# jeun-990806/pim-jpeg-decoder

Measured on AMD Instinct MI355X. Metric: MPixels/sec JPEG->RGB (bit-exact BMP), higher is better.
Workload: dtype int16/int32 (integer IDCT), u8 out

## Files before the change

### pim-jpeg-decoder_amd/csrc/pjd_k_huffman.hip

```cpp
#include <cstdlib>

#include "pjd_device_common.h"
#include "pjd_kernels.h"
#include "pjd_lut_build.h"
#include "../../include/pjd.h"

static_assert(sizeof(PjdDevHuffRaw) == 180, "raw table layout");
static_assert(PJD_LUT_BITS + PJD_L2_BITS == 16 && PJD_L1_BYTES == (4 << PJD_LUT_BITS), "two-level table geometry");
static_assert(PJD_HUFF_LANES == 64, "one wave per 64 lanes");
static_assert(PJD_STAGE_ENTRIES == PJD_GROUP && PJD_GROUP == 16, "a group (a head word + 7 step words) is what one flush of the staging buffer writes");

__global__ __launch_bounds__(256) void pjd_k_build_tables(PjdDevBatch B)
{
    const uint32_t ts = blockIdx.x / PJD_MAX_TABLES, slot = blockIdx.x % PJD_MAX_TABLES;
    const PjdDevTset &T = B.tsets[ts];
    if (slot >= T.n_tables || T.lut_bytes == 0) return;
    const PjdDevHuffRaw &r = B.raw_tables[(size_t)ts * PJD_MAX_TABLES + slot];
    uint16_t *blob = reinterpret_cast<uint16_t *>(B.luts + (size_t)T.lut_off16 * 16);
    uint32_t *L1 = reinterpret_cast<uint32_t *>(blob + slot * (PJD_L1_BYTES / 2));
    const uint32_t partner = r.is_ac ? slot : (uint32_t)T.pair_ac[slot];
    const bool has_partner = partner < T.n_tables;
    const PjdDevHuffRaw &r2 = B.raw_tables[(size_t)ts * PJD_MAX_TABLES + (has_partner ? partner : slot)];
    __shared__ uint32_t first[17], first2[17];
    __shared__ uint16_t cp[PJD_L2_BITS], ce[PJD_L2_BITS];
// ... 16 lines not shown

struct __attribute__((packed)) UnalignedU32x4 { uint32_t v[4]; };

__global__ __launch_bounds__(256) void pjd_k_lane_words(PjdDevBatch B)
{
    const uint32_t wv = blockIdx.x;
    const PjdDevHuffWave hw = B.hwaves[wv];
    const PjdDevImage &im = B.images[hw.image];
    const uint32_t l = threadIdx.x & 63, k0 = threadIdx.x >> 6;
    const uint32_t rows = PJD_WORD_ROWS(im.sub_bytes);
    uint32_t *dst = B.words + (size_t)wv * B.word_rows * 64;
    const bool valid = l < hw.n_lanes;
    const uint8_t *src = B.ecs + im.ecs_off + (valid ? B.lanes[hw.first_lane + l].byte_start : 0u);
#if PJD_WORDS_X4
    for (uint32_t k = 4 * k0; k < rows; k += 16) {
        uint32_t w[4] = {0, 0, 0, 0};
        if (valid) {
            const UnalignedU32x4 v = *reinterpret_cast<const UnalignedU32x4 *>(src + 4 * k);
#pragma unroll
            for (int j = 0; j < 4; j++) w[j] = __builtin_bswap32(v.v[j]);
        }
#pragma unroll
        for (int j = 0; j < 4; j++) dst[(k + j) * 64 + l] = w[j];
    }
#else
    for (uint32_t k = k0; k < rows; k += 4) {
        uint32_t w = 0;
        if (valid) w = __builtin_bswap32(reinterpret_cast<const UnalignedU32 *>(src + 4 * k)->v);
        dst[k * 64 + l] = w;
    }
#endif
}

typedef const __attribute__((address_space(1))) uint8_t *pjd_gptr;
#if PJD_DIRECT_ECS
#define PJD_WORD_STRIDE 4u
#else
#define PJD_WORD_STRIDE 256u
#endif
struct BitWin {
    pjd_gptr wb;
    uint32_t hi, lo, nxt;
    uint32_t off;
    int s;
    __device__ __forceinline__ uint32_t word(uint32_t byte_off) const
    {
#if PJD_DIRECT_ECS
        return __builtin_bswap32(reinterpret_cast<const __attribute__((address_space(1))) UnalignedU32 *>(wb + byte_off)->v);
#else
        return *reinterpret_cast<const __attribute__((address_space(1))) uint32_t *>(wb + byte_off);
#endif
    }
    __device__ __forceinline__ void init(pjd_gptr wave_words, uint32_t col, uint32_t p)
    {
        wb = wave_words;
        const int kk = (int)((p + 31) >> 5) - 1;
        const uint32_t o = (uint32_t)(kk + 1) * PJD_WORD_STRIDE + col;
        hi = kk >= 0 ? word(o - PJD_WORD_STRIDE) : 0u;
        lo = word(o);
        nxt = word(o + PJD_WORD_STRIDE);
        off = o + 2 * PJD_WORD_STRIDE;
        s = 32 * (kk + 1) - (int)p;
    }
    __device__ __forceinline__ uint32_t peek() const { return __builtin_amdgcn_alignbit(hi, lo, (uint32_t)s); }
    __device__ __forceinline__ void drop(uint32_t n)
    {
// ... 78 lines not shown
    __device__ __forceinline__ void build(uint32_t lane) const
    {
        if (lane <= dus1) {
            const uint32_t rn = next(lane), cn = comp(rn);
            uint4 rec;
            rec.x = tabs(rn);
            rec.y = xbase + rn * 16;
            rec.z = cn == 0 ? 0x0000ffffu : (cn == 1 ? 0xffff0000u : 0u);
            rec.w = cn == 2 ? 0x0000ffffu : 0u;
            pjd_v4u32 v; v.x = rec.x; v.y = rec.y; v.z = rec.z; v.w = rec.w;
            *reinterpret_cast<__attribute__((address_space(3))) pjd_v4u32 *>(xbase + lane * 16) = v;
        }
    }
    __device__ __forceinline__ uint32_t self(uint32_t r) const { return xbase + (r == dus1 ? 0u : r + 1) * 16; }
};

struct ChkCtx {
    uint32_t *state;
    uint32_t *rem;
    uint32_t chk_bits;
    uint32_t walk_max;
};

enum { SPAN_END = 0, SPAN_MERGED = 1, SPAN_MERGED_B = 2 };

struct BCache {
    uint32_t st;
    uint32_t rem;
    uint32_t p, cz;
};

__device__ __forceinline__ void chk_finish(const ChkCtx &K, uint32_t j, uint32_t ndu)
{
    for (uint32_t i = 1; i < j; i++) K.rem[i * 64] = ndu - K.rem[i * 64];
}

__device__ __forceinline__ uint32_t lut_lookup_pair(uint32_t lbase, uint32_t tab, uint32_t pk)
{
    uint32_t e = lds_u32(tab + 4 * __builtin_amdgcn_ubfe(pk, 32 - PJD_LUT_BITS, PJD_LUT_BITS));
    if (__builtin_expect(PJD_LUT_USED(e) == 0, 0)) {
        e = lds_u16(lbase + PJD_LUT_PTR_BYTES(e) + 2u * ((pk << PJD_LUT_BITS) >> PJD_LUT_PTR_SHIFT(e)));
        e |= e << 16;
    }
    return e;
}
__device__ __forceinline__ uint32_t lut_lookup(uint32_t lbase, uint32_t tab, uint32_t pk) { return lut_lookup_pair(lbase, tab, pk) & 0xffffu; }

__device__ __forceinline__ uint32_t rfl(uint32_t v) { return (uint32_t)__builtin_amdgcn_readfirstlane((int)v); }

__device__ __forceinline__ uint32_t add_flag(uint32_t v, bool f)
{
    uint32_t d;
    asm("v_addc_co_u32_e64 %0, vcc, %1, 0, %2" : "=v"(d) : "v"(v), "s"(__builtin_amdgcn_ballot_w64(f)) : "vcc");
    return d;
}

template <bool BRIDGE>
__device__ __forceinline__ int sync_span(const PhaseCtx &P, pjd_gptr wave_words, uint32_t col,
                                         uint32_t &p, uint32_t &c, uint32_t &z, uint32_t end_bit,
                                         uint32_t &ndu, const ChkCtx &K, uint32_t &jout, uint32_t Bst, uint32_t &oldA_st, uint32_t &oldA_rem)
{
    uint32_t j = 1;
    jout = 1;
    oldA_st = 0xffffffffu; oldA_rem = 0;
    if (p >= end_bit) return SPAN_END;
    BitWin2 w;
    w.init(wave_words, col, p);
    uint32_t ra, x;
    {
        const uint2 cur = lds_u32x2(P.self(P.dus1 - c));
        x = cur.x; ra = cur.y;
    }
    int zb = 63 - (int)z;
    uint32_t next_chk = K.chk_bits;
    uint32_t lim = next_chk < end_bit ? next_chk : end_bit;
    int res = SPAN_END;
    auto step = [&](uint32_t pk) -> bool {
        const uint2 nx = lds_u32x2(ra);
        const uint32_t tab = (zb == 63) ? (x & 0xffffu) : (x >> 16);
        const uint32_t e = lut_lookup_pair(P.lbase, tab, pk);
        const uint32_t u1 = PJD_LUT_USED(e), u12 = PJD_LUT_PAIR_USED(e);
// ... 134 lines not shown
            st = (63u << 8) | (st & 0xffu);
            if ((st & 0x80u) || second) break;
            second = true; Ddc = DdcB; Dac = DacB; Edc = e2; Eac = e3;
        }
#undef WALK_FIX
#undef WALK_PTR
        zb = (int)(st >> 8);
        const uint32_t k = (st & 0xffu) - bias;
        p += k;
        if (p >= lim) {
            if (p >= end_bit) break;
            const uint32_t st = (p << 14) | (r << 10) | (uint32_t)zb;
            const uint32_t a = rfl(st_col[j * 64]);
            if (a == st) { ndu += rfl(rem_col[j * 64]); res = SPAN_MERGED; break; }
            if (j == 1) {
                oldA_st = a; oldA_rem = rfl(rem_col[64]);
                if (st == Bst) { res = SPAN_MERGED_B; break; }
            }
            if (l == 0) { st_col[j * 64] = st; rem_col[j * 64] = ndu; }
            j++;
            next_chk += chk_bits;
            lim = next_chk < end_bit ? next_chk : end_bit;
        }
    }
    c = dus1 - r;
    z = 63u - (uint32_t)zb;
    jout = j;
    return res;
#undef WALK_TABS
#undef WALK_NEXT
}

struct OutCtx {
    uint16_t *region;
    uint32_t *stage;
    uint32_t cap;
    uint32_t n;
    uint32_t npair;
    uint32_t dcA, dcB;
    uint32_t mark_D;
    uint32_t ru;
    PjdDevMark *marks;
    uint32_t mark_next;
    uint32_t lane_q;
    uint32_t overflow;
    uint32_t D_in;
};

__device__ __forceinline__ void stage_flush(const OutCtx &O, uint32_t first_slot)
{
    uint4 *dst = reinterpret_cast<uint4 *>(O.region + first_slot);
#pragma unroll
    for (int k = 0; k < PJD_STAGE_ENTRIES / 8; k++) {
        uint4 v;
        v.x = O.stage[(4 * k + 0) * 64]; v.y = O.stage[(4 * k + 1) * 64];
        v.z = O.stage[(4 * k + 2) * 64]; v.w = O.stage[(4 * k + 3) * 64];
        dst[k] = v;
    }
}

struct WState {
    uint32_t p;
    int zb;
    uint32_t ra, x;
    uint32_t mA, mB;
    uint32_t emax;
    uint32_t umin;
};

typedef unsigned short pjd_u16x2 __attribute__((ext_vector_type(2)));
__device__ __forceinline__ uint32_t pk_add16(uint32_t a, uint32_t b)
{
    return __builtin_bit_cast(uint32_t, (pjd_u16x2)(__builtin_bit_cast(pjd_u16x2, a) + __builtin_bit_cast(pjd_u16x2, b)));
}

__device__ __forceinline__ int jpeg_extend(uint32_t bits, uint32_t size)
{
    const uint32_t m1 = 1u << size;
    return (int)bits + ((((int)bits - (int)(m1 >> 1)) >> 31) & (int)(1u - m1));
}
__device__ __forceinline__ int jpeg_value(uint32_t pk, uint32_t used, uint32_t size)
{
    const uint32_t off = 32u - used;
    const uint32_t b = __builtin_amdgcn_ubfe(pk, off, size);
    const uint32_t m = (1u << size) - 1u;
    const uint32_t top = (uint32_t)__builtin_amdgcn_sbfe(pk, off + size - 1u, 1u);
    return (int)(b - (m & ~top));
}

template <bool FIRST>
__device__ __forceinline__ uint32_t write_step(uint32_t lbase, BitWin2 &w, WState &S, uint32_t &D, OutCtx &O, uint32_t end_bit)
{
    const bool is_dc = (S.zb == 63);
    if (__builtin_expect(is_dc && D == O.mark_D, 0)) {
        PjdDevMark m;
        m.lane = O.lane_q; m.ent_off = O.n;
        m.acc[0] = (uint16_t)O.dcA; m.acc[1] = (uint16_t)(O.dcA >> 16); m.acc[2] = (uint16_t)O.dcB; m.pad_ = 0;
        O.marks[O.mark_next++] = m;
        O.mark_D += O.ru;
    }
    const uint32_t pk = FIRST ? w.peek0() : w.peek1();
    const uint4 nx = lds_u32x4(S.ra);
    const uint32_t tab = is_dc ? (S.x & 0xffffu) : (S.x >> 16);
    const uint32_t e = lut_lookup_pair(lbase, tab, pk);
    const uint32_t u1 = PJD_LUT_USED(e), size1 = PJD_LUT_SIZE(e), adv1 = PJD_LUT_ADV(e);
    const uint32_t u12 = PJD_LUT_PAIR_USED(e), adv12 = PJD_LUT_PAIR_ADV(e), size2 = PJD_LUT_PAIR_SIZE2(e);
    const bool pair = u12 != u1 && S.zb >= (int)adv1 && S.p + u1 < end_bit;
    O.npair += pair ? 1u : 0u;
    const int val1 = jpeg_value(pk, u1, size1);
    const int val2 = jpeg_value(pk, u12, size2);
    const uint32_t used = pair ? u12 : u1, adv = pair ? adv12 : adv1;
    w.drop(used);
    S.p += used;
    { const uint32_t el = e & 0xffffu; S.emax = S.emax > el ? S.emax : el; }
    S.zb -= (int)adv;
    const bool done = S.zb < 0;
    { const uint32_t u = (uint32_t)(S.zb + 16); S.umin = S.umin < u ? S.umin : u; }
    const uint32_t entA = is_dc ? (uint32_t)val1 : (((uint32_t)val1 << 5) | (adv1 & 31u));
    const uint32_t entB = pair ? (((uint32_t)val2 << 5) | ((adv12 - adv1) & 31u)) : PJD_ENT_NONE;
    const uint32_t dv = is_dc ? ((uint32_t)val1 & 0xffffu) : 0u;
    const uint32_t dvv = dv | (dv << 16);
    O.dcA = pk_add16(O.dcA, dvv & S.mA);
    O.dcB = pk_add16(O.dcB, dvv & S.mB);
    S.zb = done ? 63 : S.zb;
    S.ra = done ? nx.y : S.ra;
    S.x = done ? nx.x : S.x;
    S.mA = done ? nx.z : S.mA;
    S.mB = done ? nx.w : S.mB;
    D = add_flag(D, done);
// ... 54 lines not shown
    uint32_t dcA, dcB;
};

__device__ __forceinline__ void careful_span(const PhaseCtx &P, pjd_gptr wave_words, uint32_t col, uint32_t p, uint32_t c, uint32_t z,
                                          uint32_t end_bit, uint32_t eof_rel, bool to_eof, uint32_t D, uint32_t D_end, uint16_t *region, uint32_t cap,
                                          Careful &R)
{
    const uint32_t D_in = D;
    uint32_t *region32 = reinterpret_cast<uint32_t *>(region);
    BitWin w;
    w.init(wave_words, col, p);
    uint4 cur = lds_u32x4(P.self(P.dus1 - c));
    int zb = 63 - (int)z;
    R.n = 0; R.ovf = 0; R.cls = 0; R.p_err = 0; R.D_err = 0; R.in_dc = 0; R.dcA = 0; R.dcB = 0;
    const bool at_end = eof_rel != 0xffffffffu;
    bool open = false;
    uint32_t open_at = 0, open_ent = 0;
    while (D < D_end && (p < end_bit || to_eof)) {
        const bool is_dc = zb == 63;
        if (!open) {
            if ((R.n & (PJD_GROUP - 1)) == 0 && R.n + 2 <= cap) {
                region32[R.n >> 1] = ((D - D_in) << 8) | (63u - (uint32_t)zb);
                R.n += 2;
            }
            if (is_dc && D == R.mark_D) {
                PjdDevMark m;
                m.lane = R.lane_q; m.ent_off = R.n;
                m.acc[0] = (uint16_t)R.dcA; m.acc[1] = (uint16_t)(R.dcA >> 16); m.acc[2] = (uint16_t)R.dcB; m.pad_ = 0;
                R.marks[R.mark_next++] = m;
                R.mark_D += R.ru;
            }
        }
        const uint32_t pk = w.peek();
        const uint4 nx = lds_u32x4(cur.y);
        const uint32_t e = lut_lookup(P.lbase, is_dc ? (cur.x & 0xffffu) : (cur.x >> 16), pk);
        const uint32_t used = PJD_LUT_USED(e), size = PJD_LUT_SIZE(e), adv = PJD_LUT_ADV(e);
        const uint32_t vbits = size >= PJD_LUT_BADSYM ? 0u : size, codelen = used - vbits;
        const uint32_t left = !at_end ? 64u : (eof_rel > p ? eof_rel - p : 0u);
        uint32_t bad = 0;
        if (size == PJD_LUT_BADSYM || codelen > left) bad = is_dc ? PJD_ST_DC_SYM : PJD_ST_AC_SYM;
        else if (is_dc) {
            if (size == PJD_LUT_BADLEN) bad = PJD_ST_DC_LEN;
            else if (vbits > left - codelen) bad = PJD_ST_DC_BITS;
        } else if (!(e & PJD_LUT_EOB)) {
            if (zb - (int)adv <= -2) bad = PJD_ST_AC_RUN;
            else if (size == PJD_LUT_BADLEN) bad = PJD_ST_AC_LEN;
            else if (vbits > left - codelen) bad = PJD_ST_AC_BITS;
        }
        if (bad) {
            R.cls = bad; R.p_err = p; R.D_err = D; R.in_dc = is_dc ? 1u : 0u;
            if (!is_dc) {
                if (open) region32[open_at] = open_ent | (PJD_ENT_EOB << 16);
                else if (R.n + 2 <= cap) { region32[R.n >> 1] = PJD_ENT_EOB | (PJD_ENT_NONE << 16); R.n += 2; }
                else R.ovf = 1;
            }
            break;
        }
        const int val = jpeg_extend(__builtin_amdgcn_ubfe(pk, 32u - used, size), size);
        w.drop(used);
        p += used;
        zb -= (int)adv;
        const bool done = zb < 0;
        const uint32_t ent = is_dc ? ((uint32_t)val & 0xffffu) : ((((uint32_t)val << 5) | (adv & 31u)) & 0xffffu);
        if (open) { region32[open_at] = open_ent | (ent << 16); open = false; }
        else if (R.n + 2 <= cap) {
            region32[R.n >> 1] = ent | (PJD_ENT_NONE << 16);
            open = !done; open_at = R.n >> 1; open_ent = ent;
            R.n += 2;
        } else R.ovf = 1;
        const uint32_t dv = is_dc ? ((uint32_t)val & 0xffffu) : 0u, dvv = dv | (dv << 16);
        R.dcA = pk_add16(R.dcA, dvv & cur.z);
        R.dcB = pk_add16(R.dcB, dvv & cur.w);
        if (done) { zb = 63; cur = nx; D++; }
    }
    if ((R.n & (PJD_GROUP - 1)) == 2) R.n -= 2;
}

struct LaneGeom {
    bool valid, seg_first, seg_last;
    uint32_t q;
    uint32_t seg;
    uint32_t end_bit;
    uint32_t seg_end_bit;
    uint32_t base_bit;
    pjd_gptr words;
    uint32_t col;
};

extern __shared__ __attribute__((aligned(16))) uint8_t pjd_huff_lds[];

struct WaveState { uint32_t p_img, cz, cnt; };

__device__ __forceinline__ bool wave_rounds(const PhaseCtx &P, const LaneGeom &g, const ChkCtx &K, WalkBuf &wb, WaveState &S, BCache &Bc, uint32_t changed,
                                            uint32_t ext_p, uint32_t ext_cz, bool ext_new, uint32_t &err_acc,
                                            unsigned long long *stats, int stat_base, uint32_t *rdbg)
{
    const uint32_t l = threadIdx.x & 63;
    for (int iter = 0; iter < PJD_SYNC_MAX_ITERS; iter++) {
#if PJD_TAIL_PRIO
        if (iter == 1) __builtin_amdgcn_s_setprio(2);
        if (iter == 4) __builtin_amdgcn_s_setprio(3);
#endif
        uint32_t pp = __shfl_up(S.p_img, 1), pcz = __shfl_up(S.cz, 1), pch = __shfl_up(changed, 1);
        if (l == 0) { pp = ext_p; pcz = ext_cz; pch = (ext_new && iter == 0) ? 1u : 0u; }
        const bool act = g.valid && !g.seg_first && pch != 0;
        const uint64_t act_mask = __ballot(act);
        if (!act_mask) return true;
        const uint64_t tr0 = rdbg ? __builtin_amdgcn_s_memrealtime() : 0;
        if ((uint32_t)__popcll(act_mask) <= K.walk_max) {
            uint64_t mask = act_mask;
            uint32_t walked = 0;
            const uint32_t chk_bits = rfl(K.chk_bits);
            const uint64_t can = __ballot(g.valid && !g.seg_first);
            while (mask) {
                uint32_t a = (uint32_t)__builtin_ctzll(mask);
                mask &= mask - 1;
                uint32_t ep = rfl(ext_p), ecz = rfl(ext_cz);
                if (a) { ep = (uint32_t)__builtin_amdgcn_readlane((int)S.p_img, (int)(a - 1)); ecz = (uint32_t)__builtin_amdgcn_readlane((int)S.cz, (int)(a - 1)); }
                for (;;) {
                    const uint32_t base = (uint32_t)__builtin_amdgcn_readlane((int)g.base_bit, (int)a);
                    const uint32_t endb = (uint32_t)__builtin_amdgcn_readlane((int)g.end_bit, (int)a);
                    uint32_t p = ep - base, c = ecz >> 8, z = ecz & 255u, ndu = 0, j;
                    uint32_t *st_col = K.state - l + a, *rem_col = K.rem - l + a;
                    const uint32_t Bst_a = (uint32_t)__builtin_amdgcn_readlane((int)Bc.st, (int)a);
                    uint32_t oa_st, oa_rem;
                    const int res = walk_lane(P, wb, l, base, p, c, z, endb, ndu, st_col, rem_col, chk_bits, j, Bst_a, oa_st, oa_rem);
                    walked++;
                    const uint32_t op = (uint32_t)__builtin_amdgcn_readlane((int)S.p_img, (int)a), ocz = (uint32_t)__builtin_amdgcn_readlane((int)S.cz, (int)a);
                    uint32_t np = p + base, ncz = (c << 8) | z;
                    if (res == SPAN_MERGED_B) {
                        const uint32_t Brem_a = (uint32_t)__builtin_amdgcn_readlane((int)Bc.rem, (int)a);
                        np = (uint32_t)__builtin_amdgcn_readlane((int)Bc.p, (int)a); ncz = (uint32_t)__builtin_amdgcn_readlane((int)Bc.cz, (int)a);
                        ndu += Brem_a;
                        if (l == 0) { st_col[64] = Bst_a; rem_col[64] = Brem_a; st_col[128] = 0xffffffffu; st_col[192] = 0xffffffffu; }
                    } else if (l == 0) for (uint32_t i = 1; i < j; i++) rem_col[i * 64] = ndu - rem_col[i * 64];
                    if (l == a) {
                        S.cnt = ndu;
                        if (oa_st != 0xffffffffu || res == SPAN_MERGED_B) { Bc.st = oa_st; Bc.rem = oa_rem; Bc.p = op; Bc.cz = ocz; }
                    }
                    if (res == SPAN_MERGED || (np == op && ncz == ocz)) break;
                    if (l == a) { S.p_img = np; S.cz = ncz; }
                    if (a == 63) break;
                    if (!((can >> (a + 1)) & 1ull)) break;
                    a++; mask &= ~(1ull << a);
                    ep = np; ecz = ncz;
                }
            }
            if (stats && l == 0) { atomicAdd(stats + stat_base, 1ull); atomicAdd(stats + stat_base + 1, (unsigned long long)walked); atomicAdd(stats + PJD_STAT_WALKS, 1ull); atomicAdd(stats + PJD_STAT_WALKS + 1, (unsigned long long)walked); }
            if (rdbg && l == 0 && iter < 24) rdbg[iter] = ((0x80u | (walked & 0x7fu)) << 24) | ((uint32_t)(__builtin_amdgcn_s_memrealtime() - tr0) & 0xffffffu);
            return true;
        }
        if (stats && l == 0) { atomicAdd(stats + stat_base, 1ull); atomicAdd(stats + stat_base + 1, (unsigned long long)__popcll(act_mask)); }
        changed = 0;
        if (act) {
            uint32_t p = pp - g.base_bit, c = pcz >> 8, z = pcz & 255, ndu = 0, j, oa_st, oa_rem;
            const int res = sync_span<true>(P, g.words, g.col, p, c, z, g.end_bit, ndu, K, j, Bc.st, oa_st, oa_rem);
            const uint32_t op = S.p_img, ocz = S.cz;
            if (res == SPAN_MERGED_B) {
                ndu += Bc.rem;
                K.state[64] = Bc.st; K.rem[64] = Bc.rem; K.state[128] = 0xffffffffu; K.state[192] = 0xffffffffu;
                if (Bc.p != S.p_img || Bc.cz != S.cz) { S.p_img = Bc.p; S.cz = Bc.cz; changed = 1; }
            } else {
                chk_finish(K, j, ndu);
                if (res != SPAN_MERGED) {
                    const uint32_t np = p + g.base_bit, ncz = (c << 8) | z;
                    if (np != S.p_img || ncz != S.cz) { S.p_img = np; S.cz = ncz; changed = 1; }
                }
            }
// ... 139 lines not shown
            const uint32_t i1 = i0 + PJD_HUFF_THREADS, i2 = i1 + PJD_HUFF_THREADS, i3 = i2 + PJD_HUFF_THREADS;
            uint4 v0 = tsrc[i0], v1, v2, v3;
            if (i1 < n16) v1 = tsrc[i1];
            if (i2 < n16) v2 = tsrc[i2];
            if (i3 < n16) v3 = tsrc[i3];
            tdst[i0] = v0;
            if (i1 < n16) tdst[i1] = v1;
            if (i2 < n16) tdst[i2] = v2;
            if (i3 < n16) tdst[i3] = v3;
        }
    }
    const bool wave_on = wi < wg.n_waves;
    const uint32_t w = wg.first_wave + (wave_on ? wi : 0u);
    const PjdDevHuffWave hw = B.hwaves[w];
    const PjdDevImage &im = B.images[hw.image];
    PhaseCtx P;
    {
        const uint32_t nl = rfl(im.n_luma), dus = rfl(im.dus_per_mcu), nc = dus - nl;
        const uint32_t c1 = nc >= 1 ? 1u : 0u, c2 = nc >= 2 ? 2u : c1;
        const uint32_t lb = lds_abs(lds);
        P.lbase = lb;
        P.tY  = rfl((lb + (uint32_t)im.tbl_slot[0][0] * PJD_L1_BYTES) | (lb + (uint32_t)im.tbl_slot[0][1] * PJD_L1_BYTES) << 16);
        P.tC1 = rfl((lb + (uint32_t)im.tbl_slot[c1][0] * PJD_L1_BYTES) | (lb + (uint32_t)im.tbl_slot[c1][1] * PJD_L1_BYTES) << 16);
        P.tC2 = rfl((lb + (uint32_t)im.tbl_slot[c2][0] * PJD_L1_BYTES) | (lb + (uint32_t)im.tbl_slot[c2][1] * PJD_L1_BYTES) << 16);
        P.nc = nc; P.dus1 = dus - 1;
        P.xbase = lds_abs(phase_tabs) + wi * PJD_PHASE_LDS;
    }
    const uint32_t dus = P.dus1 + 1;
    P.build(l);
    __syncthreads();
    if (!wave_on) return;
    if (B.pull) __builtin_amdgcn_s_setprio(1);

    const uint64_t ts0 = B.dbg ? __builtin_amdgcn_s_memrealtime() : 0;
    const uint64_t tc0 = B.dbg ? __builtin_amdgcn_s_memtime() : 0;
    uint64_t *genA = B.wave_gen, *genB = B.wave_gen + B.n_hwave;
    LaneGeom g;
    g.valid = l < hw.n_lanes;
    g.q = hw.first_lane + l;
    g.seg_first = g.seg_last = false;
    g.seg = 0; g.end_bit = g.seg_end_bit = g.base_bit = 0;
#if PJD_DIRECT_ECS
    g.words = (pjd_gptr)readfirstlane_u64((uint64_t)(B.ecs + im.ecs_off));
    g.col = 0;
#else
    g.words = (pjd_gptr)readfirstlane_u64((uint64_t)(B.words + (size_t)w * B.word_rows * 64));
    g.col = l * 4;
#endif
    uint32_t seg_first_du = 0, seg_n_du = 0;
    const uint32_t sub_bytes = rfl(im.sub_bytes);
    if (g.valid) {
        const PjdDevSub sb = B.lanes[g.q];
        g.seg = sb.seg & 0x7fffffffu;
        g.seg_first = (sb.seg >> 31) != 0;
        const PjdDevSegment sg = B.segs[g.seg];
        const uint32_t end_byte = sb.byte_start + sub_bytes < sg.byte_end ? sb.byte_start + sub_bytes : sg.byte_end;
        g.seg_last = end_byte == sg.byte_end;
        g.base_bit = sb.byte_start * 8;
#if PJD_DIRECT_ECS
        g.col = sb.byte_start;
#endif
        g.end_bit = (end_byte - sb.byte_start) * 8;
        g.seg_end_bit = (sg.byte_end - sb.byte_start) * 8;
        seg_first_du = sg.first_du; seg_n_du = sg.n_du;
    }
    uint32_t *area = reinterpret_cast<uint32_t *>(areas + wi * PJD_WAVE_LDS);
    ChkCtx K;
    K.state = area + l;
    K.rem = area + PJD_NCHK * 64 + l;
    K.chk_bits = sub_bytes * 8 / PJD_NCHK;
    K.walk_max = rfl(im.walk_max);
    for (int j = 0; j < PJD_NCHK; j++) { K.state[j * 64] = 0xffffffffu; K.rem[j * 64] = 0; }
    const bool first_is_head = __shfl((uint32_t)g.seg_first, 0) != 0;
    const uint32_t last_lane = hw.n_lanes - 1;
    bool dead = false;
    uint32_t flag = 0;

    WaveState S;
    {
        uint32_t p = 0, c = 0, z = 0, ndu = 0, j = 1;
        if (g.valid) {
            uint32_t oa, orem;
            sync_span<false>(P, g.words, g.col, p, c, z, g.end_bit, ndu, K, j, 0xffffffffu, oa, orem);
            chk_finish(K, j, ndu);
        }
        S.p_img = p + g.base_bit; S.cz = (c << 8) | z; S.cnt = ndu;
    }
    if (l == last_lane) op_store(genA + w, pjd_pack_state(S.p_img, S.cz >> 8, S.cz & 255) | OP_FLAG);
    const uint64_t ts1 = B.dbg ? __builtin_amdgcn_s_memrealtime() : 0;

    uint64_t entry_used = 0;
    uint32_t err_acc = 0;
    bool ok = true;
    WalkBuf wb;
    wb.ecs = (pjd_gptr)readfirstlane_u64((uint64_t)(B.ecs + im.ecs_off));
    wb.clamp = rfl(im.ecs_len) + 40u;
    wb.cb = 0; wb.cw = 0; wb.cn = 0; wb.have = 0;
    if (!first_is_head) entry_used = op_wait_flag(genA + w - 1, dead);
    BCache Bc;
    Bc.st = 0xffffffffu; Bc.rem = 0; Bc.p = 0; Bc.cz = 0;
    ok = wave_rounds(P, g, K, wb, S, Bc, g.valid ? 1u : 0u, (uint32_t)entry_used,
                     (((uint32_t)(entry_used >> 32) & 255) << 8) | ((uint32_t)(entry_used >> 40) & 255), !first_is_head && !dead,
                     err_acc, B.stats, 0, B.dbg ? B.dbg + (size_t)w * 32 + 8 : nullptr);
    if (l == last_lane) op_store(genB + w, pjd_pack_state(S.p_img, S.cz >> 8, S.cz & 255) | OP_FLAG);
    const uint64_t ts2 = B.dbg ? __builtin_amdgcn_s_memrealtime() : 0;

    for (uint32_t gen = 1; gen + 1 < PJD_GENS; gen++) {
        if (!first_is_head && !dead) {
            const uint64_t truth = op_wait_flag(B.wave_gen + (size_t)gen * B.n_hwave + w - 1, dead);
            if (!dead && truth != entry_used) {
                entry_used = truth;
                ok = wave_rounds(P, g, K, wb, S, Bc, 0u, (uint32_t)truth,
                                 (((uint32_t)(truth >> 32) & 255) << 8) | ((uint32_t)(truth >> 40) & 255), true,
                                 err_acc, B.stats, 2, nullptr) && ok;
            }
        }
        if (l == last_lane) op_store(B.wave_gen + (size_t)(gen + 1) * B.n_hwave + w, pjd_pack_state(S.p_img, S.cz >> 8, S.cz & 255) | OP_FLAG);
    }
    if (!ok) flag |= 1u << PJD_FLAG_NOSYNC;
    const uint64_t ts3 = B.dbg ? __builtin_amdgcn_s_memrealtime() : 0;

    const uint32_t du_cap = rfl(im.n_du) + 1;
    uint32_t cnt = 0, v = 0, f = 0;
    if (g.valid) {
        cnt = S.cnt;
        v = cnt < du_cap ? cnt : du_cap;
        if (g.seg_first) { f = 1; v = seg_first_du + v < du_cap ? seg_first_du + v : du_cap; }
    }
    wave_seg_scan(v, f, du_cap);
    const uint32_t agg_v = __shfl(v, 63), agg_f = __shfl(f, 63);
    uint32_t du_in = 0;
    if (w == im.hwave_base) {
        if (l == 0) op_store(B.wave_desc + w, op_desc(OP_ST_PFX, agg_v, agg_f, dead));
    } else {
        if (l == 0) op_store(B.wave_desc + w, op_desc(OP_ST_AGG, agg_v, agg_f, dead));
        uint32_t rv = 0, rf = 0;
        bool poison = false;
        int hi = (int)w - 1;
        for (;;) {
            const int j = hi - (int)l;
            const bool inside = j >= (int)im.hwave_base;
            uint64_t d = OP_ST_PFX;
            if (inside) {
                uint32_t it = 0;
                do { d = op_load(B.wave_desc + j); if (d & OP_ST_MASK) break; __builtin_amdgcn_s_sleep(8); } while (++it < OP_SPIN_LIMIT);
            }
            const bool ready = (d & OP_ST_MASK) != 0;
            if (__any(!ready)) { dead = true; break; }
            const uint64_t pfx_mask = __ballot((d & OP_ST_MASK) == OP_ST_PFX);
            const int k = pfx_mask ? __builtin_ctzll(pfx_mask) : 64;
            const bool use = (int)l <= k;
            uint32_t xv = use ? (uint32_t)d & 0x0fffffffu : 0u, xf = use ? (uint32_t)((d >> 60) & 1u) : 0u;
            poison = poison || __any(use && (d & OP_POISON));
            for (int off = 1; off < 64; off <<= 1) {
                const uint32_t ov = __shfl_down(xv, off), of = __shfl_down(xf, off);
                if ((int)l + off < 64) seg_combine(ov, of, xv, xf, du_cap);
            }
            const uint32_t wvv = __shfl(xv, 0), wf = __shfl(xf, 0);
            { uint32_t nv = rv, nf = rf; seg_combine(wvv, wf, nv, nf, du_cap); rv = nv; rf = nf; }
            if (k < 64) break;
            hi -= 64;
        }
        if (poison) dead = true;
        du_in = rv;
        uint32_t iv = agg_v, ifl = agg_f;
        seg_combine(rv, rf, iv, ifl, du_cap);
        if (l == 0) op_store(B.wave_desc + w, op_desc(OP_ST_PFX, iv, ifl, dead));
    }
    const uint64_t ts4 = B.dbg ? __builtin_amdgcn_s_memrealtime() : 0;

    const uint32_t prev_p = __shfl_up(S.p_img, 1), prev_cz = __shfl_up(S.cz, 1);
    const uint32_t prev_v = __shfl_up(v, 1), prev_f = __shfl_up(f, 1);
    uint32_t npair = 0;
    PjdDevLaneInfo li;
    li.n_ent = 0; li.first_du = g.seg_first ? PJD_LANE_SEG_FIRST : 0u; li.dc_sum[0] = li.dc_sum[1] = li.dc_sum[2] = 0; li.pad_ = 0;
    if (g.valid && !dead) {
        uint32_t D;
        if (g.seg_first) D = seg_first_du;
        else if (l == 0) D = du_in;
        else if (prev_f) D = prev_v;
        else D = du_in + prev_v < du_cap ? du_in + prev_v : du_cap;
        const uint32_t D_in = D, D_end = seg_first_du + seg_n_du;
        uint32_t p, c, z;
        if (g.seg_first) { p = 0; c = 0; z = 0; }
        else {
            if (l == 0) { p = (uint32_t)entry_used - g.base_bit; c = (uint32_t)(entry_used >> 32) & 255; z = (uint32_t)(entry_used >> 40) & 255; }
            else { p = prev_p - g.base_bit; c = prev_cz >> 8; z = prev_cz & 255; }
            if (D_in < D_end && (D_in % dus) != c) flag |= 1u << PJD_FLAG_SEGMENT;
        }
        if (D_in < D_end && !flag) {
            OutCtx O;
            O.region = B.ent + im.ent_base + (size_t)(g.q - im.lane_base) * im.lane_cap;
            O.stage = area + l;
            O.cap = im.lane_cap;
            O.n = 0; O.npair = 0; O.dcA = 0; O.dcB = 0; O.overflow = 0;
            O.ru = im.idct_mcus * dus;
            O.marks = B.marks + im.iwg_base;
            O.lane_q = g.q;
            O.D_in = D_in;
            li.first_du |= D_in;
            {
                const uint32_t first_du = im.first_mcu * dus;
                const uint32_t d_next = (z == 0) ? D_in : D_in + 1;
                const uint32_t k = (d_next - first_du + O.ru - 1) / O.ru;
                O.mark_next = k;
                O.mark_D = first_du + k * O.ru;
            }
            uint32_t err = 0;
            const uint32_t p0 = p, c0 = c, z0 = z, mark_next0 = O.mark_next, mark_D0 = O.mark_D;
            write_span(P, g.words, g.col, p, c, z, g.end_bit, err, D, D_end, O);
            li.n_ent = O.n;
            npair = O.npair;
            li.dc_sum[0] = (uint16_t)O.dcA; li.dc_sum[1] = (uint16_t)(O.dcA >> 16); li.dc_sum[2] = (uint16_t)O.dcB;
            const bool has_next = g.seg + 1 < im.seg_base + im.n_seg;
            const bool last_seg = !has_next && (im.flags & PJD_IF_ENDS_STREAM) != 0;
            const bool eof_lane = g.seg_last && last_seg;
            const bool eof_crossed = last_seg && !g.seg_last && p > g.seg_end_bit;
            bool settled = false;
            if (err || (eof_lane && (D < D_end || p > g.seg_end_bit)) || eof_crossed) {
                Careful R;
                R.marks = O.marks; R.mark_next = mark_next0; R.mark_D = mark_D0; R.ru = O.ru; R.lane_q = g.q;
                careful_span(P, g.words, g.col, p0, c0, z0, g.end_bit, (eof_lane || eof_crossed) ? g.seg_end_bit : 0xffffffffu, eof_lane,
                             D_in, D_end, O.region, O.cap, R);
                li.n_ent = R.n;
                npair = 0;
                li.dc_sum[0] = (uint16_t)R.dcA; li.dc_sum[1] = (uint16_t)(R.dcA >> 16); li.dc_sum[2] = (uint16_t)R.dcB;
                if (R.ovf) flag |= 1u << PJD_FLAG_OVERFLOW;
                else if (R.cls) {
                    const unsigned long long key = ((unsigned long long)(g.base_bit + R.p_err) << 32) | ((unsigned long long)R.D_err << 4) | (R.cls << 1) | R.in_dc;
                    atomicMin(&B.imstate[hw.image].err_key, key);
                    settled = true;
                }
            }
            if (!settled) {
                if (err) flag |= 1u << PJD_FLAG_SYMBOL;
                if (O.overflow) flag |= 1u << PJD_FLAG_OVERFLOW;
                if (D == D_end) {
                    if (p > g.seg_end_bit) flag |= 1u << PJD_FLAG_SEGMENT;
                    if (has_next && ((p + 7) & ~7u) != g.seg_end_bit) flag |= 1u << PJD_FLAG_SEGMENT;
                } else {
                    if (S.p_img - g.base_bit != p || (S.cz >> 8) != c || (S.cz & 255) != z) flag |= 1u << PJD_FLAG_VERIFY;
                    if (D - D_in != S.cnt) flag |= 1u << PJD_FLAG_VERIFY;
                    if (g.seg_last) flag |= 1u << PJD_FLAG_SEGMENT;
                }
            }
        }
    }
    if (g.valid) B.lane_info[g.q] = li;
    if (!first_is_head && !dead) {
        const uint64_t fin = op_wait_flag(B.wave_gen + (size_t)(PJD_GENS - 1) * B.n_hwave + w - 1, dead);
        if (fin != entry_used) flag |= 1u << PJD_FLAG_STITCH;
    }
    if (B.dbg && l == 0) {
        const uint64_t ts5 = __builtin_amdgcn_s_memrealtime();
        uint32_t *d = B.dbg + (size_t)w * 32;
        d[0] = (uint32_t)ts0; d[1] = (uint32_t)(ts1 - ts0); d[2] = (uint32_t)(ts2 - ts1); d[3] = (uint32_t)(ts3 - ts2);
        d[4] = (uint32_t)(ts4 - ts3); d[5] = (uint32_t)(ts5 - ts4); d[6] = hw.image; d[7] = hw.n_lanes;
        d[7] |= ((uint32_t)(((__builtin_amdgcn_s_memtime() - tc0) * 16) / ((ts5 - ts0) ? (ts5 - ts0) : 1)) & 0xffffffu) << 8;
    }
    if (dead) flag |= 1u << PJD_FLAG_TIMEOUT;
    uint32_t wflag = flag, went = npair, wsteps = g.valid ? li.n_ent / 2 - (li.n_ent + PJD_GROUP - 1) / PJD_GROUP : 0, wpos = (flag && g.valid) ? g.base_bit : 0xffffffffu;
    uint32_t wfill = g.valid ? (uint32_t)(((uint64_t)li.n_ent << 10) / im.lane_cap) : 0u;
    for (int off = 1; off < 64; off <<= 1) {
        wflag |= __shfl_xor(wflag, off); went += __shfl_xor(went, off); wsteps += __shfl_xor(wsteps, off);
        { const uint32_t o = __shfl_xor(wfill, off); wfill = o > wfill ? o : wfill; }
        const uint32_t o = __shfl_xor(wpos, off);
        wpos = o < wpos ? o : wpos;
    }
    if (l == 0) { atomicAdd(B.stats + PJD_STAT_ENTRIES, (unsigned long long)(went + wsteps)); atomicAdd(B.stats + PJD_STAT_STEPS, (unsigned long long)wsteps); atomicMax(B.stats + PJD_STAT_FILL, (unsigned long long)wfill); }
    if (wflag && l == 0) {
        atomicMin(&B.imstate[hw.image].flag_pos, wpos);
        for (int r = 0; r < PJD_FLAG_REASONS; r++)
            if (wflag & (1u << r)) atomicAdd(B.stats + PJD_STAT_FLAG0 + r, 1ull);
    }
    if (B.pull) {
        __atomic_thread_fence(__ATOMIC_RELEASE);
        uint32_t done = 0;
        if (l == 0) done = atomicAdd(&B.imstate[hw.image].waves_done, 1u) + 1u;
        if (rfl(done) == rfl(im.n_hwave)) finish_picture(B, hw.image, l);
    }
}

struct SeqWin {
    pjd_gptr base;
    uint32_t hi, lo, nxt, off;
    int s;
    __device__ __forceinline__ uint32_t word(uint32_t byte_off) const
    {
        return __builtin_bswap32(reinterpret_cast<const __attribute__((address_space(1))) UnalignedU32 *>(base + byte_off)->v);
    }
    __device__ __forceinline__ void init(pjd_gptr b)
    {
        base = b; hi = 0; lo = word(0); nxt = word(4); off = 8; s = 0;
    }
    __device__ __forceinline__ uint32_t peek() const { return __builtin_amdgcn_alignbit(hi, lo, (uint32_t)s); }
// ... 128 lines not shown
```

Before: 143,400.

## Cut live registers in Huffman wave kernel by rematerializing lane geometry

Removes many per-lane values (segment index, seg_end_bit, seg_last, lane q, original start state, 64-bit debug timestamps) from the long-lived state. It reloads them from global memory after the write span, or recomputes them from lane_id and shuffles. The output pointer becomes a wave-uniform base plus a per-lane offset, the careful-path restart state is recovered with shuffles, and prefetching of the next descriptor in careful_span is deferred. The aim is lower VGPR/SGPR pressure and less spilling in the hot decode loop, at the cost of extra global reloads and a wave-wide check before the careful path.

```diff
diff --git a/pim-jpeg-decoder_amd/csrc/pjd_k_huffman.hip b/pim-jpeg-decoder_amd/csrc/pjd_k_huffman.hip
--- a/pim-jpeg-decoder_amd/csrc/pjd_k_huffman.hip
+++ b/pim-jpeg-decoder_amd/csrc/pjd_k_huffman.hip
@@ -72,6 +72,7 @@
 #endif
 }
 
+typedef __attribute__((address_space(1))) uint8_t *pjd_gwptr;
 typedef const __attribute__((address_space(1))) uint8_t *pjd_gptr;
 #if PJD_DIRECT_ECS
 #define PJD_WORD_STRIDE 4u
@@ -216,6 +217,7 @@
 
 __device__ __forceinline__ void chk_finish(const ChkCtx &K, uint32_t j, uint32_t ndu)
 {
+#pragma nounroll
     for (uint32_t i = 1; i < j; i++) K.rem[i * 64] = ndu - K.rem[i * 64];
 }
 
@@ -231,6 +233,7 @@
 __device__ __forceinline__ uint32_t lut_lookup(uint32_t lbase, uint32_t tab, uint32_t pk) { return lut_lookup_pair(lbase, tab, pk) & 0xffffu; }
 
 __device__ __forceinline__ uint32_t rfl(uint32_t v) { return (uint32_t)__builtin_amdgcn_readfirstlane((int)v); }
+__device__ __forceinline__ uint32_t lane_id() { return __builtin_amdgcn_mbcnt_hi(~0u, __builtin_amdgcn_mbcnt_lo(~0u, 0u)); }
 
 __device__ __forceinline__ uint32_t add_flag(uint32_t v, bool f)
 {
@@ -431,7 +434,8 @@
 }
 
 struct OutCtx {
-    uint16_t *region;
+    pjd_gwptr ent0;
+    uint32_t roff;
     uint32_t *stage;
     uint32_t cap;
     uint32_t n;
@@ -441,17 +445,17 @@
     uint32_t ru;
     PjdDevMark *marks;
     uint32_t mark_next;
-    uint32_t lane_q;
+    uint32_t lane_q0;
     uint32_t overflow;
     uint32_t D_in;
 };
 
 __device__ __forceinline__ void stage_flush(const OutCtx &O, uint32_t first_slot)
 {
-    uint4 *dst = reinterpret_cast<uint4 *>(O.region + first_slot);
+    __attribute__((address_space(1))) pjd_v4u32 *dst = reinterpret_cast<__attribute__((address_space(1))) pjd_v4u32 *>(O.ent0 + (O.roff + 2u * first_slot));
 #pragma unroll
     for (int k = 0; k < PJD_STAGE_ENTRIES / 8; k++) {
-        uint4 v;
+        pjd_v4u32 v;
         v.x = O.stage[(4 * k + 0) * 64]; v.y = O.stage[(4 * k + 1) * 64];
         v.z = O.stage[(4 * k + 2) * 64]; v.w = O.stage[(4 * k + 3) * 64];
         dst[k] = v;
@@ -493,7 +497,7 @@
     const bool is_dc = (S.zb == 63);
     if (__builtin_expect(is_dc && D == O.mark_D, 0)) {
         PjdDevMark m;
-        m.lane = O.lane_q; m.ent_off = O.n;
+        m.lane = O.lane_q0 + lane_id(); m.ent_off = O.n;
         m.acc[0] = (uint16_t)O.dcA; m.acc[1] = (uint16_t)(O.dcA >> 16); m.acc[2] = (uint16_t)O.dcB; m.pad_ = 0;
         O.marks[O.mark_next++] = m;
         O.mark_D += O.ru;
@@ -614,7 +618,6 @@
             }
         }
         const uint32_t pk = w.peek();
-        const uint4 nx = lds_u32x4(cur.y);
         const uint32_t e = lut_lookup(P.lbase, is_dc ? (cur.x & 0xffffu) : (cur.x >> 16), pk);
         const uint32_t used = PJD_LUT_USED(e), size = PJD_LUT_SIZE(e), adv = PJD_LUT_ADV(e);
         const uint32_t vbits = size >= PJD_LUT_BADSYM ? 0u : size, codelen = used - vbits;
@@ -653,21 +656,35 @@
         const uint32_t dv = is_dc ? ((uint32_t)val & 0xffffu) : 0u, dvv = dv | (dv << 16);
         R.dcA = pk_add16(R.dcA, dvv & cur.z);
         R.dcB = pk_add16(R.dcB, dvv & cur.w);
-        if (done) { zb = 63; cur = nx; D++; }
+        if (done) { zb = 63; cur = lds_u32x4(cur.y); D++; }
     }
     if ((R.n & (PJD_GROUP - 1)) == 2) R.n -= 2;
 }
 
 struct LaneGeom {
-    bool valid, seg_first, seg_last;
-    uint32_t q;
-    uint32_t seg;
+    bool valid, seg_first;
     uint32_t end_bit;
-    uint32_t seg_end_bit;
     uint32_t base_bit;
     pjd_gptr words;
     uint32_t col;
 };
+
+struct LanePlan {
+    uint32_t byte_start;
+    uint32_t seg;
+    bool seg_first;
+    PjdDevSegment sg;
+};
+__device__ __forceinline__ LanePlan lane_plan(const PjdDevBatch &B, uint32_t q)
+{
+    const PjdDevSub sb = B.lanes[q];
+    LanePlan r;
+    r.byte_start = sb.byte_start;
+    r.seg = sb.seg & 0x7fffffffu;
+    r.seg_first = (sb.seg >> 31) != 0;
+    r.sg = B.segs[r.seg];
+    return r;
+}
 
 extern __shared__ __attribute__((aligned(16))) uint8_t pjd_huff_lds[];
 
@@ -715,7 +732,10 @@
                         np = (uint32_t)__builtin_amdgcn_readlane((int)Bc.p, (int)a); ncz = (uint32_t)__builtin_amdgcn_readlane((int)Bc.cz, (int)a);
                         ndu += Brem_a;
                         if (l == 0) { st_col[64] = Bst_a; rem_col[64] = Brem_a; st_col[128] = 0xffffffffu; st_col[192] = 0xffffffffu; }
-                    } else if (l == 0) for (uint32_t i = 1; i < j; i++) rem_col[i * 64] = ndu - rem_col[i * 64];
+                    } else if (l == 0) {
+#pragma nounroll
+                        for (uint32_t i = 1; i < j; i++) rem_col[i * 64] = ndu - rem_col[i * 64];
+                    }
                     if (l == a) {
                         S.cnt = ndu;
                         if (oa_st != 0xffffffffu || res == SPAN_MERGED_B) { Bc.st = oa_st; Bc.rem = oa_rem; Bc.p = op; Bc.cz = ocz; }
@@ -921,14 +941,23 @@
     if (!wave_on) return;
     if (B.pull) __builtin_amdgcn_s_setprio(1);
 
-    const uint64_t ts0 = B.dbg ? __builtin_amdgcn_s_memrealtime() : 0;
-    const uint64_t tc0 = B.dbg ? __builtin_amdgcn_s_memtime() : 0;
+    uint32_t *const dbg_row = B.dbg ? B.dbg + (size_t)w * 32 : nullptr;
+    uint32_t ts_prev = 0;
+    if (dbg_row) {
+        ts_prev = (uint32_t)__builtin_amdgcn_s_memrealtime();
+        if (l == 0) { dbg_row[0] = ts_prev; dbg_row[7] = (uint32_t)__builtin_amdgcn_s_memtime(); }
+    }
+#define PJD_DBG_STAMP(k_)                                                                                               \
+    if (dbg_row) {                                                                                                      \
+        const uint32_t now_ = (uint32_t)__builtin_amdgcn_s_memrealtime();                                               \
+        if (l == 0) dbg_row[k_] = now_ - ts_prev;                                                                       \
+        ts_prev = now_;                                                                                                 \
+    }
     uint64_t *genA = B.wave_gen, *genB = B.wave_gen + B.n_hwave;
     LaneGeom g;
     g.valid = l < hw.n_lanes;
-    g.q = hw.first_lane + l;
-    g.seg_first = g.seg_last = false;
-    g.seg = 0; g.end_bit = g.seg_end_bit = g.base_bit = 0;
+    g.seg_first = false;
+    g.end_bit = g.base_bit = 0;
 #if PJD_DIRECT_ECS
     g.words = (pjd_gptr)readfirstlane_u64((uint64_t)(B.ecs + im.ecs_off));
     g.col = 0;
@@ -936,22 +965,17 @@
     g.words = (pjd_gptr)readfirstlane_u64((uint64_t)(B.words + (size_t)w * B.word_rows * 64));
     g.col = l * 4;
 #endif
-    uint32_t seg_first_du = 0, seg_n_du = 0;
     const uint32_t sub_bytes = rfl(im.sub_bytes);
+    const uint32_t lane_q0 = rfl(hw.first_lane);
     if (g.valid) {
-        const PjdDevSub sb = B.lanes[g.q];
-        g.seg = sb.seg & 0x7fffffffu;
-        g.seg_first = (sb.seg >> 31) != 0;
-        const PjdDevSegment sg = B.segs[g.seg];
-        const uint32_t end_byte = sb.byte_start + sub_bytes < sg.byte_end ? sb.byte_start + sub_bytes : sg.byte_end;
-        g.seg_last = end_byte == sg.byte_end;
-        g.base_bit = sb.byte_start * 8;
+        const LanePlan lp = lane_plan(B, lane_q0 + l);
+        const uint32_t end_byte = lp.byte_start + sub_bytes < lp.sg.byte_end ? lp.byte_start + sub_bytes : lp.sg.byte_end;
+        g.seg_first = lp.seg_first;
+        g.base_bit = lp.byte_start * 8;
 #if PJD_DIRECT_ECS
-        g.col = sb.byte_start;
+        g.col = lp.byte_start;
 #endif
-        g.end_bit = (end_byte - sb.byte_start) * 8;
-        g.seg_end_bit = (sg.byte_end - sb.byte_start) * 8;
-        seg_first_du = sg.first_du; seg_n_du = sg.n_du;
+        g.end_bit = (end_byte - lp.byte_start) * 8;
     }
     uint32_t *area = reinterpret_cast<uint32_t *>(areas + wi * PJD_WAVE_LDS);
     ChkCtx K;
@@ -976,7 +1000,7 @@
         S.p_img = p + g.base_bit; S.cz = (c << 8) | z; S.cnt = ndu;
     }
     if (l == last_lane) op_store(genA + w, pjd_pack_state(S.p_img, S.cz >> 8, S.cz & 255) | OP_FLAG);
-    const uint64_t ts1 = B.dbg ? __builtin_amdgcn_s_memrealtime() : 0;
+    PJD_DBG_STAMP(1)
 
     uint64_t entry_used = 0;
     uint32_t err_acc = 0;
@@ -990,9 +1014,9 @@
     Bc.st = 0xffffffffu; Bc.rem = 0; Bc.p = 0; Bc.cz = 0;
     ok = wave_rounds(P, g, K, wb, S, Bc, g.valid ? 1u : 0u, (uint32_t)entry_used,
                      (((uint32_t)(entry_used >> 32) & 255) << 8) | ((uint32_t)(entry_used >> 40) & 255), !first_is_head && !dead,
-                     err_acc, B.stats, 0, B.dbg ? B.dbg + (size_t)w * 32 + 8 : nullptr);
+                     err_acc, B.stats, 0, dbg_row ? dbg_row + 8 : nullptr);
     if (l == last_lane) op_store(genB + w, pjd_pack_state(S.p_img, S.cz >> 8, S.cz & 255) | OP_FLAG);
-    const uint64_t ts2 = B.dbg ? __builtin_amdgcn_s_memrealtime() : 0;
+    PJD_DBG_STAMP(2)
 
     for (uint32_t gen = 1; gen + 1 < PJD_GENS; gen++) {
         if (!first_is_head && !dead) {
@@ -1007,11 +1031,14 @@
         if (l == last_lane) op_store(B.wave_gen + (size_t)(gen + 1) * B.n_hwave + w, pjd_pack_state(S.p_img, S.cz >> 8, S.cz & 255) | OP_FLAG);
     }
     if (!ok) flag |= 1u << PJD_FLAG_NOSYNC;
-    const uint64_t ts3 = B.dbg ? __builtin_amdgcn_s_memrealtime() : 0;
+    PJD_DBG_STAMP(3)
 
     const uint32_t du_cap = rfl(im.n_du) + 1;
     uint32_t cnt = 0, v = 0, f = 0;
+    uint32_t seg_first_du = 0, D_end = 0;
     if (g.valid) {
+        const LanePlan lp = lane_plan(B, lane_q0 + lane_id());
+        seg_first_du = lp.sg.first_du; D_end = seg_first_du + lp.sg.n_du;
         cnt = S.cnt;
         v = cnt < du_cap ? cnt : du_cap;
         if (g.seg_first) { f = 1; v = seg_first_du + v < du_cap ? seg_first_du + v : du_cap; }
@@ -1056,21 +1083,34 @@
         seg_combine(rv, rf, iv, ifl, du_cap);
         if (l == 0) op_store(B.wave_desc + w, op_desc(OP_ST_PFX, iv, ifl, dead));
     }
-    const uint64_t ts4 = B.dbg ? __builtin_amdgcn_s_memrealtime() : 0;
+    PJD_DBG_STAMP(4)
 
     const uint32_t prev_p = __shfl_up(S.p_img, 1), prev_cz = __shfl_up(S.cz, 1);
     const uint32_t prev_v = __shfl_up(v, 1), prev_f = __shfl_up(f, 1);
     uint32_t npair = 0;
     PjdDevLaneInfo li;
-    li.n_ent = 0; li.first_du = g.seg_first ? PJD_LANE_SEG_FIRST : 0u; li.dc_sum[0] = li.dc_sum[1] = li.dc_sum[2] = 0; li.pad_ = 0;
+    li.n_ent = 0; li.first_du = 0; li.dc_sum[0] = li.dc_sum[1] = li.dc_sum[2] = 0; li.pad_ = 0;
+    const uint32_t end_bit = g.end_bit;
+    const bool valid = g.valid;
+    const uint32_t want_p = S.p_img, want_czn = S.cz | (S.cnt << 16);
+    const uint32_t ru = rfl(im.idct_mcus) * dus, first_mark_du = rfl(im.first_mcu) * dus;
+    auto first_mark = [&](uint32_t D_in, uint32_t z) { return ((z == 0 ? D_in : D_in + 1) - first_mark_du + ru - 1) / ru; };
+    bool ran = false;
+    uint32_t p = 0, c = 0, z = 0, D = 0, D_in = 0, err = 0;
+    OutCtx O;
+    O.ent0 = (pjd_gwptr)readfirstlane_u64((uint64_t)(B.ent + im.ent_base + (size_t)(hw.first_lane - im.lane_base) * im.lane_cap));
+    O.cap = rfl(im.lane_cap);
+    O.roff = l * O.cap * 2u;
+    O.ru = ru;
+    O.marks = B.marks + rfl(im.iwg_base);
+    O.lane_q0 = lane_q0;
+    O.n = 0; O.npair = 0; O.dcA = 0; O.dcB = 0; O.overflow = 0;
     if (g.valid && !dead) {
-        uint32_t D;
         if (g.seg_first) D = seg_first_du;
         else if (l == 0) D = du_in;
         else if (prev_f) D = prev_v;
         else D = du_in + prev_v < du_cap ? du_in + prev_v : du_cap;
-        const uint32_t D_in = D, D_end = seg_first_du + seg_n_du;
-        uint32_t p, c, z;
+        D_in = D;
         if (g.seg_first) { p = 0; c = 0; z = 0; }
         else {
             if (l == 0) { p = (uint32_t)entry_used - g.base_bit; c = (uint32_t)(entry_used >> 32) & 255; z = (uint32_t)(entry_used >> 40) & 255; }
@@ -1078,78 +1118,83 @@
             if (D_in < D_end && (D_in % dus) != c) flag |= 1u << PJD_FLAG_SEGMENT;
         }
         if (D_in < D_end && !flag) {
-            OutCtx O;
-            O.region = B.ent + im.ent_base + (size_t)(g.q - im.lane_base) * im.lane_cap;
             O.stage = area + l;
-            O.cap = im.lane_cap;
-            O.n = 0; O.npair = 0; O.dcA = 0; O.dcB = 0; O.overflow = 0;
-            O.ru = im.idct_mcus * dus;
-            O.marks = B.marks + im.iwg_base;
-            O.lane_q = g.q;
             O.D_in = D_in;
-            li.first_du |= D_in;
-            {
-                const uint32_t first_du = im.first_mcu * dus;
-                const uint32_t d_next = (z == 0) ? D_in : D_in + 1;
-                const uint32_t k = (d_next - first_du + O.ru - 1) / O.ru;
-                O.mark_next = k;
-                O.mark_D = first_du + k * O.ru;
-            }
-            uint32_t err = 0;
-            const uint32_t p0 = p, c0 = c, z0 = z, mark_next0 = O.mark_next, mark_D0 = O.mark_D;
-            write_span(P, g.words, g.col, p, c, z, g.end_bit, err, D, D_end, O);
+            O.mark_next = first_mark(D_in, z);
+            O.mark_D = first_mark_du + O.mark_next * ru;
+            write_span(P, g.words, g.col, p, c, z, end_bit, err, D, D_end, O);
+            ran = true;
             li.n_ent = O.n;
             npair = O.npair;
             li.dc_sum[0] = (uint16_t)O.dcA; li.dc_sum[1] = (uint16_t)(O.dcA >> 16); li.dc_sum[2] = (uint16_t)O.dcB;
-            const bool has_next = g.seg + 1 < im.seg_base + im.n_seg;
-            const bool last_seg = !has_next && (im.flags & PJD_IF_ENDS_STREAM) != 0;
-            const bool eof_lane = g.seg_last && last_seg;
-            const bool eof_crossed = last_seg && !g.seg_last && p > g.seg_end_bit;
-            bool settled = false;
-            if (err || (eof_lane && (D < D_end || p > g.seg_end_bit)) || eof_crossed) {
-                Careful R;
-                R.marks = O.marks; R.mark_next = mark_next0; R.mark_D = mark_D0; R.ru = O.ru; R.lane_q = g.q;
-                careful_span(P, g.words, g.col, p0, c0, z0, g.end_bit, (eof_lane || eof_crossed) ? g.seg_end_bit : 0xffffffffu, eof_lane,
-                             D_in, D_end, O.region, O.cap, R);
-                li.n_ent = R.n;
-                npair = 0;
-                li.dc_sum[0] = (uint16_t)R.dcA; li.dc_sum[1] = (uint16_t)(R.dcA >> 16); li.dc_sum[2] = (uint16_t)R.dcB;
-                if (R.ovf) flag |= 1u << PJD_FLAG_OVERFLOW;
-                else if (R.cls) {
-                    const unsigned long long key = ((unsigned long long)(g.base_bit + R.p_err) << 32) | ((unsigned long long)R.D_err << 4) | (R.cls << 1) | R.in_dc;
-                    atomicMin(&B.imstate[hw.image].err_key, key);
-                    settled = true;
-                }
-            }
-            if (!settled) {
-                if (err) flag |= 1u << PJD_FLAG_SYMBOL;
-                if (O.overflow) flag |= 1u << PJD_FLAG_OVERFLOW;
-                if (D == D_end) {
-                    if (p > g.seg_end_bit) flag |= 1u << PJD_FLAG_SEGMENT;
-                    if (has_next && ((p + 7) & ~7u) != g.seg_end_bit) flag |= 1u << PJD_FLAG_SEGMENT;
-                } else {
-                    if (S.p_img - g.base_bit != p || (S.cz >> 8) != c || (S.cz & 255) != z) flag |= 1u << PJD_FLAG_VERIFY;
-                    if (D - D_in != S.cnt) flag |= 1u << PJD_FLAG_VERIFY;
-                    if (g.seg_last) flag |= 1u << PJD_FLAG_SEGMENT;
-                }
-            }
-        }
-    }
-    if (g.valid) B.lane_info[g.q] = li;
+        }
+    }
+    struct { uint32_t base_bit, seg_end_bit, col; bool seg_first, seg_last, has_next; } tl = {0, 0, 0, false, false, false};
+    const uint32_t q = lane_q0 + lane_id();
+    if (valid) {
+        const LanePlan lp = lane_plan(B, q);
+        tl.base_bit = lp.byte_start * 8;
+        tl.col = PJD_DIRECT_ECS ? lp.byte_start : 4u * lane_id();
+        tl.seg_end_bit = (lp.sg.byte_end - lp.byte_start) * 8;
+        tl.seg_first = lp.seg_first;
+        tl.seg_last = lp.byte_start + sub_bytes >= lp.sg.byte_end;
+        tl.has_next = lp.seg + 1 < im.seg_base + im.n_seg;
+    }
+    li.first_du = (tl.seg_first ? PJD_LANE_SEG_FIRST : 0u) | (ran ? D_in : 0u);
+    const bool last_seg = !tl.has_next && (im.flags & PJD_IF_ENDS_STREAM) != 0;
+    const bool eof_lane = tl.seg_last && last_seg;
+    const bool eof_crossed = last_seg && !tl.seg_last && p > tl.seg_end_bit;
+    const bool careful = ran && (err || (eof_lane && (D < D_end || p > tl.seg_end_bit)) || eof_crossed);
+    bool settled = false;
+    if (__any(careful)) {
+        uint32_t p0 = __shfl_up(want_p, 1), cz0 = __shfl_up(want_czn, 1) & 0xffffu;
+        if (l == 0) { p0 = (uint32_t)entry_used; cz0 = (((uint32_t)(entry_used >> 32) & 255) << 8) | ((uint32_t)(entry_used >> 40) & 255); }
+        if (careful) {
+            uint32_t c0 = cz0 >> 8, z0 = cz0 & 255u;
+            p0 -= tl.base_bit;
+            if (tl.seg_first) { p0 = 0; c0 = 0; z0 = 0; }
+            Careful R;
+            R.marks = O.marks; R.mark_next = first_mark(D_in, z0); R.mark_D = first_mark_du + R.mark_next * ru; R.ru = ru; R.lane_q = q;
+            careful_span(P, g.words, tl.col, p0, c0, z0, end_bit, (eof_lane || eof_crossed) ? tl.seg_end_bit : 0xffffffffu, eof_lane,
+                         D_in, D_end, (uint16_t *)(O.ent0 + O.roff), O.cap, R);
+            li.n_ent = R.n;
+            npair = 0;
+            li.dc_sum[0] = (uint16_t)R.dcA; li.dc_sum[1] = (uint16_t)(R.dcA >> 16); li.dc_sum[2] = (uint16_t)R.dcB;
+            if (R.ovf) flag |= 1u << PJD_FLAG_OVERFLOW;
+            else if (R.cls) {
+                const unsigned long long key = ((unsigned long long)(tl.base_bit + R.p_err) << 32) | ((unsigned long long)R.D_err << 4) | (R.cls << 1) | R.in_dc;
+                atomicMin(&B.imstate[hw.image].err_key, key);
+                settled = true;
+            }
+        }
+    }
+    if (ran && !settled) {
+        if (err) flag |= 1u << PJD_FLAG_SYMBOL;
+        if (O.overflow) flag |= 1u << PJD_FLAG_OVERFLOW;
+        if (D == D_end) {
+            if (p > tl.seg_end_bit) flag |= 1u << PJD_FLAG_SEGMENT;
+            if (tl.has_next && ((p + 7) & ~7u) != tl.seg_end_bit) flag |= 1u << PJD_FLAG_SEGMENT;
+        } else {
+            if (want_p - tl.base_bit != p || (want_czn & 0xffffu) != ((c << 8) | z)) flag |= 1u << PJD_FLAG_VERIFY;
+            if (D - D_in != want_czn >> 16) flag |= 1u << PJD_FLAG_VERIFY;
+            if (tl.seg_last) flag |= 1u << PJD_FLAG_SEGMENT;
+        }
+    }
+    if (valid) B.lane_info[q] = li;
     if (!first_is_head && !dead) {
         const uint64_t fin = op_wait_flag(B.wave_gen + (size_t)(PJD_GENS - 1) * B.n_hwave + w - 1, dead);
         if (fin != entry_used) flag |= 1u << PJD_FLAG_STITCH;
     }
-    if (B.dbg && l == 0) {
-        const uint64_t ts5 = __builtin_amdgcn_s_memrealtime();
-        uint32_t *d = B.dbg + (size_t)w * 32;
-        d[0] = (uint32_t)ts0; d[1] = (uint32_t)(ts1 - ts0); d[2] = (uint32_t)(ts2 - ts1); d[3] = (uint32_t)(ts3 - ts2);
-        d[4] = (uint32_t)(ts4 - ts3); d[5] = (uint32_t)(ts5 - ts4); d[6] = hw.image; d[7] = hw.n_lanes;
-        d[7] |= ((uint32_t)(((__builtin_amdgcn_s_memtime() - tc0) * 16) / ((ts5 - ts0) ? (ts5 - ts0) : 1)) & 0xffffffu) << 8;
+    PJD_DBG_STAMP(5)
+#undef PJD_DBG_STAMP
+    if (dbg_row && l == 0) {
+        const uint32_t span = ts_prev - dbg_row[0], cyc = (uint32_t)__builtin_amdgcn_s_memtime() - dbg_row[7];
+        dbg_row[6] = hw.image;
+        dbg_row[7] = hw.n_lanes | ((uint32_t)(((uint64_t)cyc * 16) / (span ? span : 1)) & 0xffffffu) << 8;
     }
     if (dead) flag |= 1u << PJD_FLAG_TIMEOUT;
-    uint32_t wflag = flag, went = npair, wsteps = g.valid ? li.n_ent / 2 - (li.n_ent + PJD_GROUP - 1) / PJD_GROUP : 0, wpos = (flag && g.valid) ? g.base_bit : 0xffffffffu;
-    uint32_t wfill = g.valid ? (uint32_t)(((uint64_t)li.n_ent << 10) / im.lane_cap) : 0u;
+    uint32_t wflag = flag, went = npair, wsteps = valid ? li.n_ent / 2 - (li.n_ent + PJD_GROUP - 1) / PJD_GROUP : 0, wpos = (flag && valid) ? tl.base_bit : 0xffffffffu;
+    uint32_t wfill = valid ?(uint32_t)(((uint64_t)li.n_ent << 10) / im.lane_cap) : 0u;
     for (int off = 1; off < 64; off <<= 1) {
         wflag |= __shfl_xor(wflag, off); went += __shfl_xor(went, off); wsteps += __shfl_xor(wsteps, off);
         { const uint32_t o = __shfl_xor(wfill, off); wfill = o > wfill ? o : wfill; }
```

Result: no change. 143,000 (-0.3%).
